# BetterBelle/eco-dqn

Measured on AMD Instinct MI355X. Metric: env-steps/sec (batched episodes) on ER-200 MaxCut, higher is better.
Workload: dtype f32-accurate MPNN on f16 MFMA (fp16x2: every operand a power-of-two-scaled pair of fp16 pieces, 22 significand bits, three products, f32 accumulate; aggregations and Linears alike; f32 MFMA on the CSR fallback) / f64+int (env)

## Files before the change

eco-dqn_amd/csrc/eco_train.hip:

```cpp
#include <cmath>

#include "eco_mpnn.h"
#include "eco_env_dev.h"

namespace eco {

struct WJob {
  const float* dY;
  const float* X1;
  const float* X2;
  int ld1, K1, ld2, K2;
  int R;
  int nO;
  int out_off;
  int out_ld;
  int out_col0;
};
constexpr int MAX_JOBS = 10;
#ifndef WGRAD_NT
#define WGRAD_NT 0
#endif
constexpr int WGRAD_WG_X = 3;
constexpr int WG_PER_JOB = 128;
constexpr int SLABS_PER_JOB = WG_PER_JOB;
constexpr int SLAB = 64 * 128;
constexpr int WROWS = 32;

struct WJobs {
  WJob j[MAX_JOBS];
  int n;
  int nwgj[MAX_JOBS];
  int first[MAX_JOBS + 1];
// ... 141 lines not shown
      if (rb + WROWS >= r1) break;
      store_tile(RB, rb + WROWS);
      __syncthreads();
      load_tile(RB, rb + 3 * WROWS);
      compute();
      __syncthreads();
    }
  }
  float* slab = slabs + ((size_t)jb * SLABS_PER_JOB + wg) * SLAB;
#pragma unroll
  for (int q = 0; q < 2; ++q) {
    const int t = w + 4 * q;
    if (t < ntile) {
      const int it = t >> 1;
#pragma unroll
      for (int k = 0; k < 16; ++k) {
        const int o = 32 * ot + (k & 3) + 8 * (k >> 2) + 4 * h;
        slab[o * 128 + 32 * it + jj] = acc[q][k];
      }
    }
  }
}

__global__ __launch_bounds__(256) void wgrad_bf3_kernel(WJobs jobs, float* slabs) {
  __shared__ __attribute__((aligned(16))) uint16_t sY[3 * 64 * WB_LD];
  __shared__ __attribute__((aligned(16))) uint16_t sX[3 * 128 * WB_LD];
  int jb = 0;
  while (jb + 1 < jobs.n && (int)blockIdx.x >= jobs.first[jb + 1]) ++jb;
  if (jobs.j[jb].K1 + jobs.j[jb].K2 > 64) wgrad_bf3_job<true>(jobs, slabs, jb, sY, sX);
  else wgrad_bf3_job<false>(jobs, slabs, jb, sY, sX);
}


__global__ void wgrad_reduce_kernel(WJobs jobs, const float* slabs, float* grad) {
  const WJob& J = jobs.j[blockIdx.y];
  const int K = J.K1 + J.K2;
  const int idx = blockIdx.x * blockDim.x + threadIdx.x;
  const int o = idx / 128, i = idx % 128;
  if (o >= J.nO || i >= K) return;
  const float* s = slabs + (size_t)blockIdx.y * SLABS_PER_JOB * SLAB + o * 128 + i;
  float acc = 0.f;
  const int nk = jobs.nwgj[blockIdx.y];
  int k = 0;
  for (; k + 8 <= nk; k += 8) {
    float v[8];
#pragma unroll
    for (int u = 0; u < 8; ++u) v[u] = s[(size_t)(k + u) * SLAB];
#pragma unroll
    for (int u = 0; u < 8; ++u) acc += v[u];
  }
  for (; k < nk; ++k) acc += s[(size_t)k * SLAB];
  grad[J.out_off + o * J.out_ld + J.out_col0 + i] = acc;
}

struct ColJob {
  const float* X;
  int R, ld, C;
  float* out;
  int out_stride;
};
struct ColJobs {
  ColJob j[4];
  int first[5];
};
__global__ void colsum_jobs_kernel(ColJobs jobs) {
  int jb = 0;
  while (jb < 3 && (int)blockIdx.x >= jobs.first[jb + 1]) ++jb;
  const ColJob& J = jobs.j[jb];
  __shared__ float red[256];
  const int c = (int)blockIdx.x - jobs.first[jb];
  float acc = 0.f;
  for (int r = threadIdx.x; r < J.R; r += 256) acc += J.X[(size_t)r * J.ld + c];
  red[threadIdx.x] = acc;
  __syncthreads();
  for (int s2 = 128; s2 > 0; s2 >>= 1) {
    if ((int)threadIdx.x < s2) red[threadIdx.x] += red[threadIdx.x + s2];
    __syncthreads();
  }
  if (threadIdx.x == 0) J.out[(size_t)c * J.out_stride] = red[0];
}

__global__ void td_kernel(const float* q_s, const float* q_tn, const int32_t* a_star, const int32_t* actions,
                          const float* rewards, const float* dones, int B, int N, float gamma, int clip,
                          float* dq, float* sqerr) {
  const size_t i = (size_t)blockIdx.x * blockDim.x + threadIdx.x;
  if (i >= (size_t)B * N) return;
  const int b = (int)(i / N), j = (int)(i - (size_t)b * N);
  int a = actions[b];
  if ((unsigned)a >= (unsigned)N) a = 0;
  if (j != a) {
    dq[i] = 0.f;
    return;
  }
  int as = a_star[b];
  if ((unsigned)as >= (unsigned)N) as = 0;
  float qt = q_tn[(size_t)b * N + as];
  if (clip && qt < 0.f) qt = 0.f;
  const float td = rewards[b] + (1.f - dones[b]) * gamma * qt;
  const float q = q_s[i];
  const float diff = q - td;
  dq[i] = 2.f * diff / (float)B;
  sqerr[b] = diff * diff;
}

__global__ void mean_kernel(const float* v, int n, float* out) {
  __shared__ float red[256];
  float acc = 0.f;
  for (int i = threadIdx.x; i < n; i += 256) acc += v[i];
  red[threadIdx.x] = acc;
  __syncthreads();
  for (int s = 128; s > 0; s >>= 1) {
    if ((int)threadIdx.x < s) red[threadIdx.x] += red[threadIdx.x + s];
    __syncthreads();
  }
  if (threadIdx.x == 0) *out = red[0] / (float)n;
}

__global__ void adam_kernel(float* p, const float* g, float* m, float* v, int n, float b1, float b2, float step_size,
                            float bc2_sqrt, float eps, float wd, float gscale) {
  const int i = blockIdx.x * blockDim.x + threadIdx.x;
  if (i >= n) return;
  float gi = gscale == 1.f ? g[i] : g[i] * gscale;
  if (wd != 0.f) gi = fmaf(wd, p[i], gi);
  const float mi = m[i] + (1.f - b1) * (gi - m[i]);
  const float vi = v[i] * b2 + (1.f - b2) * gi * gi;
  m[i] = mi;
  v[i] = vi;
  const float denom = sqrtf(vi) / bc2_sqrt + eps;
  p[i] = p[i] - step_size * (mi / denom);
}

__device__ __forceinline__ int xstride(const eco_replay& rb) { return rb.x_stride == 16 ? 16 : 8; }

__global__ void replay_push_kernel(eco_replay rb, int pos, int B, const float* xs, const float* xn,
                                   const int32_t* gids, const int32_t* actions, const double* rewards,
                                   const uint8_t* dones) {
  const int b = blockIdx.y;
  if (b >= B) return;
  const int slot = (int)(((long long)pos + b) % rb.capacity);
  const int per = rb.n_spins * xstride(rb) / 4;
  const float4* s4 = reinterpret_cast<const float4*>(xs + (size_t)b * rb.n_spins * xstride(rb));
  const float4* n4 = reinterpret_cast<const float4*>(xn + (size_t)b * rb.n_spins * xstride(rb));
  float4* ds = reinterpret_cast<float4*>(rb.xs + (size_t)slot * rb.n_spins * xstride(rb));
  float4* dn = reinterpret_cast<float4*>(rb.xn + (size_t)slot * rb.n_spins * xstride(rb));
  for (int i = blockIdx.x * blockDim.x + threadIdx.x; i < per; i += gridDim.x * blockDim.x) {
    ds[i] = s4[i];
    dn[i] = n4[i];
  }
  if (blockIdx.x == 0 && threadIdx.x == 0) {
    rb.gid[slot] = gids[b];
    rb.act[slot] = actions[b];
    rb.rew[slot] = (float)rewards[b];
    rb.done[slot] = dones[b] ? 1.f : 0.f;
  }
}

__device__ __forceinline__ uint32_t feistel(uint32_t x, int half, uint64_t key) {
  const uint32_t mask = (1u << half) - 1u;
  uint32_t L = x >> half, R = x & mask;
#pragma unroll
  for (int r = 0; r < 4; ++r) {
    const uint32_t F = (uint32_t)(rng3(key, (uint64_t)r, (uint64_t)R) & mask);
// ... 191 lines not shown
      const uint32_t tsfk = v == a ? 0u : (((w >> 16) & 0x7FFFu) + 1u) & 0x7FFFu;
      w = ((v == a ? ~w : w) & 0x80000000u) | (tsfk << 16) | (w & 0xFFFFu);
    }
    cr_lds[v] = w;
  }
  __syncthreads();
  if (flip) {
    const int32_t* rp = gs.row_ptr + (size_t)g * (N + 1);
    const uint32_t* ed = gs.edges + gs.edge_base[g];
    for (int q = rp[a] + threadIdx.x; q < rp[a + 1]; q += blockDim.x) {
      const uint32_t ex = ed[q];
      const int j = edge_col(ex);
      const uint32_t w = cr_lds[j];
      const int h = (int)(int16_t)(w & 0xFFFFu) - 2 * edge_w(ex) * sa_old;
      cr_lds[j] = (w & 0xFFFF0000u) | ((uint32_t)h & 0xFFFFu);
    }
    __syncthreads();
  }
  compact_expand(cfg, cr_lds, r.ctx_n + slot * 4, mlr, tab, N, xn + (size_t)m * N * W, red);
}

static size_t slab_bytes() { return (size_t)MAX_JOBS * SLABS_PER_JOB * SLAB * sizeof(float); }

}

using namespace eco;

extern "C" size_t eco_mpnn_backward_workspace_bytes(int32_t n_spins, int32_t batch) {
  const size_t g = mpnn_grad_ws_bytes(n_spins, batch);
  if (!g) return 0;
  return align_up(g, 256) + slab_bytes();
}

extern "C" int eco_mpnn_backward(const float* packed, int32_t n_obs_in, const eco_graph_set* gs,
                                 const int32_t* graph_ids, int32_t batch, const float* obs_x, const void* saved,
                                 const float* dq, float* grad, void* workspace, eco_stream_t stream) {
  if (!grad || !workspace) return fail(ECO_ERR_ARG, "null grad/workspace");
  hipStream_t st = (hipStream_t)stream;
  int rc = mpnn_backward_launch(packed, n_obs_in, gs, graph_ids, batch, obs_x, saved, dq, workspace, st);
  if (rc) return rc;
  const int N = gs->n_spins;
  const size_t RT = (size_t)batch * N;
  if (RT > (size_t)INT32_MAX / 64) return fail(ECO_ERR_ARG, "batch * n_spins too large");
  const float* sv = (const float*)saved;
  const float* gr = (const float*)workspace;
  auto SV = [&](int t) { return sv + (size_t)t * RT * 64; };
  auto GR = [&](int t) { return gr + (size_t)t * RT * 64; };
  const float* MEAN = sv + (size_t)SV_NODE_TENSORS * RT * 64;
  const float* DP = gr + (size_t)GR_NODE_TENSORS * RT * 64;
  const float* DWRA = DP + (size_t)batch * 64;
  const float* DWRB = DWRA + (size_t)batch * 64;
  const float* DBR = DWRB + (size_t)batch * 64;
  const float* DWA = DBR + (((size_t)batch + 63) & ~63ull);
  const int gpb = graphs_per_block(N, batch);
  const int nblk = (batch + gpb - 1) / gpb;
  float* slabs = (float*)((char*)workspace + align_up(mpnn_grad_ws_bytes(N, batch), 256));
  const FlatOffsets fo = flat_offsets(n_obs_in);
  WJobs J{};
  int n = 0;
  const int R = (int)RT;
  for (int l = 0; l < 3; ++l) {
    J.j[n++] = WJob{GR(GR_DUM0 + l), SV(SV_AGG0 + l), SV(SV_E), 64, 64, 64, 64, R, 64, fo.L + l * 16384, 128, 0};
    J.j[n++] = WJob{GR(GR_DUU0 + l), SV(SV_H0 + l), SV(SV_M0 + l), 64, 64, 64, 64, R, 64, fo.L + l * 16384 + 8192,
                    128, 0};
  }
  J.j[n++] = WJob{GR(GR_DUE), SV(SV_EAGG), nullptr, 64, 64, 0, 0, R, 64, fo.Wf, 64, 0};
  const int xw = ECO_OBS_X_STRIDE(n_obs_in);
  J.j[n++] = WJob{GR(GR_DU0), obs_x, nullptr, xw, n_obs_in, 0, 0, R, 64, fo.W0, n_obs_in, 0};
  J.j[n++] = WJob{GR(GR_DZ), obs_x, nullptr, xw, n_obs_in, 0, 0, R, 63, fo.We, 1 + n_obs_in, 1};
  J.j[n++] = WJob{DP, MEAN, nullptr, 64, 64, 0, 0, batch, 64, fo.Wp, 64, 0};
  J.n = n;
  {
    const int total = WGRAD_WG_X * 256;
    double rows = 0.0;
    for (int j = 0; j < n; ++j) rows += J.j[j].R;
    J.first[0] = 0;
    for (int j = 0; j < n; ++j) {
      const int g = (int)(total * (double)J.j[j].R / rows);
      J.nwgj[j] = std::max(1, std::min(WG_PER_JOB, g));
      J.first[j + 1] = J.first[j] + J.nwgj[j];
    }
    wgrad_bf3_kernel<<<J.first[n], 256, 0, st>>>(J, slabs);
  }
  wgrad_reduce_kernel<<<dim3(64 * 128 / 256, n), 256, 0, st>>>(J, slabs, grad);
  ColJobs CJ{};
  CJ.j[0] = ColJob{DWRA, batch, 64, 64, grad + fo.Wr, 1};
  CJ.j[1] = ColJob{DWRB, batch, 64, 64, grad + fo.Wr + 64, 1};
  CJ.j[2] = ColJob{DBR, batch, 1, 1, grad + fo.Br, 1};
  CJ.j[3] = ColJob{DWA, nblk, 64, 63, grad + fo.We, 1 + n_obs_in};
  CJ.first[0] = 0;
  for (int k = 0; k < 4; ++k) CJ.first[k + 1] = CJ.first[k] + CJ.j[k].C;
  colsum_jobs_kernel<<<CJ.first[4], 256, 0, st>>>(CJ);
  return check_launch("mpnn_backward_wgrad");
}

extern "C" int eco_dqn_td(const float* q_s, const float* q_target_next, const int32_t* a_star,
                          const int32_t* actions, const float* rewards, const float* dones, int32_t batch,
                          int32_t n_spins, float gamma, int32_t clip_q_targets, float* dq, float* sqerr,
                          float* loss, eco_stream_t stream) {
  if (!q_s || !q_target_next || !a_star || !actions || !rewards || !dones || !dq || !sqerr || !loss)
    return fail(ECO_ERR_ARG, "null argument");
  if (batch < 1 || n_spins < 1) return fail(ECO_ERR_ARG, "bad batch/n_spins");
  hipStream_t st = (hipStream_t)stream;
  const size_t n = (size_t)batch * n_spins;
  td_kernel<<<(unsigned)((n + 255) / 256), 256, 0, st>>>(q_s, q_target_next, a_star, actions, rewards, dones, batch,
                                                         n_spins, gamma, clip_q_targets, dq, sqerr);
  mean_kernel<<<1, 256, 0, st>>>(sqerr, batch, loss);
  return check_launch("dqn_td");
}

extern "C" int eco_adam(float* params, const float* grad, float* exp_avg, float* exp_avg_sq, int32_t n, double lr,
                        double beta1, double beta2, double eps, double weight_decay, double grad_scale, int64_t step,
                        eco_stream_t stream) {
  if (!params || !grad || !exp_avg || !exp_avg_sq || n < 1 || step < 1) return fail(ECO_ERR_ARG, "bad adam args");
  const double bc1 = 1.0 - std::pow(beta1, (double)step);
  const double bc2 = 1.0 - std::pow(beta2, (double)step);
  adam_kernel<<<(n + 255) / 256, 256, 0, (hipStream_t)stream>>>(params, grad, exp_avg, exp_avg_sq, n, (float)beta1,
                                                               (float)beta2, (float)(lr / bc1),
                                                               (float)std::sqrt(bc2), (float)eps,
                                                               (float)weight_decay, (float)grad_scale);
  return check_launch("adam");
}

extern "C" int eco_replay_push(const eco_replay* rb, int32_t pos, int32_t batch, const float* xs, const float* xn,
                               const int32_t* graph_ids, const int32_t* actions, const double* rewards,
                               const uint8_t* dones, eco_stream_t stream) {
  if (!rb || !xs || !xn || !graph_ids || !actions || !rewards || !dones) return fail(ECO_ERR_ARG, "null argument");
  if (rb->x_stride != 0 && rb->x_stride != 8 && rb->x_stride != 16) return fail(ECO_ERR_ARG, "x_stride must be 8 or 16");
  if (batch < 1 || rb->capacity < 1 || pos < 0) return fail(ECO_ERR_ARG, "bad batch/capacity/pos");
  if (batch > rb->capacity) return fail(ECO_ERR_ARG, "replay push: batch larger than the ring (slots would collide)");
  replay_push_kernel<<<dim3(1, batch), 256, 0, (hipStream_t)stream>>>(*rb, pos, batch, xs, xn, graph_ids, actions,
                                                                      rewards, dones);
  return check_launch("replay_push");
}

extern "C" int eco_replay_sample(const eco_replay* rb, int32_t size, int32_t m, uint64_t seed, uint64_t counter,
                                 float* xs, float* xn, int32_t* graph_ids, int32_t* actions, float* rewards,
                                 float* dones, eco_stream_t stream) {
  if (!rb || !xs || !xn || !graph_ids || !actions || !rewards || !dones) return fail(ECO_ERR_ARG, "null argument");
  if (rb->x_stride != 0 && rb->x_stride != 8 && rb->x_stride != 16) return fail(ECO_ERR_ARG, "x_stride must be 8 or 16");
  if (size < m || m < 1 || size > rb->capacity)
    return fail(ECO_ERR_ARG, "replay sample: need m <= size <= capacity (random.sample without replacement)");
  replay_sample_kernel<<<dim3(1, m), 256, 0, (hipStream_t)stream>>>(*rb, size, m, rng3(seed, counter, 0x5A5A),
                                                                    xs, xn, graph_ids, actions, rewards, dones);
  return check_launch("replay_sample");
}

static int compact_check(const eco_env_config* cfg, int32_t batch, int32_t capacity) {
  if (!cfg) return fail(ECO_ERR_ARG, "null config");
  if (cfg->optimisation_target != ECO_TARGET_CUT) return fail(ECO_ERR_TARGET, "compact replay: OptimisationTarget.CUT only");
  if (cfg->float_weights)
    return fail(ECO_ERR_ARG, "compact replay: integer weights only (its local field is an int16); a float-weighted "
                             "env uses the feature ring (eco_replay_push / eco_replay_sample)");
// ... 61 lines not shown
```

eco-dqn_amd/eco_hip/_lib.py:

```python
import ctypes
import os

_HERE = os.path.dirname(os.path.abspath(__file__))
LIB_PATH = os.environ.get("ECO_HIP_LIB", os.path.join(_HERE, "libecohip.so"))

if not os.path.exists(LIB_PATH):
    raise ImportError(f"libecohip.so not found at {LIB_PATH}: build it with `make -C eco-dqn_amd` "
                      "(hipcc --offload-arch=gfx950); eco_hip has no fallback path")
lib = ctypes.CDLL(LIB_PATH)

ECO_OK, ECO_ERR_ARG, ECO_ERR_HIP, ECO_ERR_PAST_END, ECO_ERR_BASIS, ECO_ERR_TARGET, ECO_ERR_OBSERVABLE, \
    ECO_ERR_GRAPH, ECO_ERR_KEY, ECO_ERR_INDEX = range(10)
ECO_MAX_OBS = 16
ECO_MPNN_MAX_OBS = 16
ECO_ENV_SCALARS = 16
ECO_TARGET_CUT, ECO_TARGET_ENERGY, ECO_TARGET_MIN_COVER, ECO_TARGET_MIN_CUT, ECO_TARGET_MAX_IND_SET, \
    ECO_TARGET_MAX_CLIQUE, ECO_TARGET_MIN_DOM_SET = range(1, 8)


def obs_x_stride(n_obs):
    return 8 if n_obs <= 8 else 16
ECO_MAX_SPINS = 2048
ECO_COMPACT_MAX_SPINS = 8192
ECO_NORM_PER_GRAPH, ECO_NORM_PER_CALL, ECO_NORM_PER_CALL_REUSE = 0, 1, 2
ECO_GRAPH_ER, ECO_GRAPH_BA = 1, 2
ECO_WEIGHTS_UNIFORM, ECO_WEIGHTS_DISCRETE, ECO_WEIGHTS_RANDOM = 0, 1, 2
ECO_PATH_NO_DENSE, ECO_PATH_NO_DL, ECO_PATH_NO_SHARED, ECO_PATH_NO_PAIR, ECO_PATH_DENSE2_FWD = 1, 2, 4, 8, 16


class EnvConfig(ctypes.Structure):
    _fields_ = [("n_spins", ctypes.c_int32), ("max_steps", ctypes.c_int32), ("n_obs", ctypes.c_int32),
                ("obs_ids", ctypes.c_int32 * ECO_MAX_OBS), ("reward_signal", ctypes.c_int32),
                ("norm_rewards", ctypes.c_int32), ("reversible_spins", ctypes.c_int32),
                ("spin_basis", ctypes.c_int32), ("stopping", ctypes.c_int32),
                ("has_basin_reward", ctypes.c_int32), ("has_stag_punishment", ctypes.c_int32),
                ("horizon_length", ctypes.c_int32), ("optimisation_target", ctypes.c_int32),
                ("basin_reward", ctypes.c_double),
                ("stag_punishment", ctypes.c_double), ("float_weights", ctypes.c_int32)]


class GraphSet(ctypes.Structure):
    _fields_ = [("n_graphs", ctypes.c_int32), ("n_spins", ctypes.c_int32), ("row_ptr", ctypes.c_void_p),
                ("edge_base", ctypes.c_void_p), ("edges", ctypes.c_void_p), ("deg", ctypes.c_void_p),
                ("max_deg", ctypes.c_void_p), ("meta", ctypes.c_void_p), ("valid", ctypes.c_void_p),
                ("unit_weights", ctypes.c_int32), ("adjbits", ctypes.c_void_p),
                ("edge_weights", ctypes.c_void_p)]


class Replay(ctypes.Structure):
    _fields_ = [("capacity", ctypes.c_int32), ("n_spins", ctypes.c_int32), ("x_stride", ctypes.c_int32),
                ("xs", ctypes.c_void_p),
                ("xn", ctypes.c_void_p), ("gid", ctypes.c_void_p), ("act", ctypes.c_void_p),
                ("rew", ctypes.c_void_p), ("done", ctypes.c_void_p)]


class ActConfig(ctypes.Structure):
    _fields_ = [("epsilon", ctypes.c_float), ("reversible", ctypes.c_int32), ("allowed_value", ctypes.c_float),
                ("seed", ctypes.c_uint64), ("counter", ctypes.c_uint64)]


_P = ctypes.c_void_p
_I = ctypes.c_int32
_SIG = {
    "eco_graphs_prepare": (ctypes.c_int, [ctypes.POINTER(GraphSet), _P]),
    "eco_graphs_adjbits_bytes": (ctypes.c_size_t, [_I, _I]),
    "eco_graphs_generate_workspace_bytes": (ctypes.c_size_t, [_I, _I]),
    "eco_graphs_generate": (ctypes.c_int, [ctypes.POINTER(GraphSet), _I, _I, _I, ctypes.c_double, _I,
                                           ctypes.c_uint64, ctypes.c_int64, _P, _P]),
    "eco_env_state_bytes": (ctypes.c_size_t, [ctypes.POINTER(EnvConfig), _I]),
    "eco_env_reset": (ctypes.c_int, [ctypes.POINTER(EnvConfig), ctypes.POINTER(GraphSet), _P, _I, _P, _P, _P,
                                     ctypes.c_uint64, _P, _P, _P]),
    "eco_env_step": (ctypes.c_int, [ctypes.POINTER(EnvConfig), ctypes.POINTER(GraphSet), _P, _I, _P, _P, _P, _P,
                                    _P, _P]),
    "eco_env_read": (ctypes.c_int, [ctypes.POINTER(EnvConfig), _P, _I, _P, _P, _P, _P]),
    "eco_check_errors": (ctypes.c_int, [_P]),
    "eco_error_word_copy": (ctypes.c_int, [_P, _P]),
    "eco_set_kernel_paths": (_I, [_I]),
    "eco_probe_split2_mfma": (ctypes.c_int, [_P, _P, _P, _I, _I, _P, _P]),
    "eco_env_greedy_actions": (ctypes.c_int, [ctypes.POINTER(EnvConfig), ctypes.POINTER(GraphSet), _P, _I, _P,
                                              _P]),
    "eco_mpnn_param_count": (ctypes.c_size_t, [_I]),
    "eco_mpnn_packed_count": (ctypes.c_size_t, []),
    "eco_mpnn_pack": (ctypes.c_int, [_P, _I, _P, _P]),
    "eco_mpnn_workspace_bytes": (ctypes.c_size_t, [_I, _I]),
    "eco_mpnn_forward": (ctypes.c_int, [_P, _I, ctypes.POINTER(GraphSet), _P, _I, _P, _I, _P,
                                        ctypes.POINTER(ActConfig), _P, _P, _P, _P]),
    "eco_mpnn_forward_pair": (ctypes.c_int, [_P, _P, _I, ctypes.POINTER(GraphSet), _P, _I, _P, _I, _P,
                                             ctypes.POINTER(ActConfig), _P, _P, ctypes.POINTER(ActConfig), _P, _P,
                                             _P]),
    "eco_mpnn_saved_bytes": (ctypes.c_size_t, [_I, _I]),
    "eco_mpnn_backward_workspace_bytes": (ctypes.c_size_t, [_I, _I]),
    "eco_mpnn_backward": (ctypes.c_int, [_P, _I, ctypes.POINTER(GraphSet), _P, _I, _P, _P, _P, _P, _P, _P]),
    "eco_dqn_td": (ctypes.c_int, [_P, _P, _P, _P, _P, _P, _I, _I, ctypes.c_float, _I, _P, _P, _P, _P]),
    "eco_adam": (ctypes.c_int, [_P, _P, _P, _P, _I, ctypes.c_double, ctypes.c_double, ctypes.c_double,
                                ctypes.c_double, ctypes.c_double, ctypes.c_double, ctypes.c_int64, _P]),
    "eco_replay_push": (ctypes.c_int, [ctypes.POINTER(Replay), _I, _I, _P, _P, _P, _P, _P, _P, _P]),
    "eco_replay_sample": (ctypes.c_int, [ctypes.POINTER(Replay), _I, _I, ctypes.c_uint64, ctypes.c_uint64, _P, _P,
                                         _P, _P, _P, _P, _P]),
    "eco_replay_compact_bytes": (ctypes.c_size_t, [_I, _I, _I]),
    "eco_replay_compact_snapshot": (ctypes.c_int, [ctypes.POINTER(EnvConfig), _P, _I, _P, _I, ctypes.c_int64, _P,
                                                   _P]),
    "eco_replay_compact_push": (ctypes.c_int, [ctypes.POINTER(EnvConfig), _P, _I, _P, _I, ctypes.c_int64, _P, _P, _P,
                                               _P]),
    "eco_replay_compact_sample": (ctypes.c_int, [ctypes.POINTER(EnvConfig), _P, ctypes.POINTER(GraphSet), _I, _P, _I,
                                                 _I, ctypes.c_int64, _I, ctypes.c_uint64, ctypes.c_uint64, _P, _P, _P, _P, _P, _P,
                                                 _P]),
    "eco_per_create": (_P, [_I, ctypes.c_double, ctypes.c_double]),
    "eco_per_destroy": (None, [_P]),
    "eco_per_len": (_I, [_P]),
    "eco_per_beta": (ctypes.c_double, [_P]),
    "eco_per_full": (ctypes.c_int, [_P]),
    "eco_per_configure_beta_anneal_time": (ctypes.c_int, [_P, ctypes.c_double]),
    "eco_per_add": (ctypes.c_int, [_P, _I, _P]),
    "eco_per_update_priorities": (ctypes.c_int, [_P, _I, _P, _P]),
    "eco_per_rebalance": (ctypes.c_int, [_P]),
    "eco_per_sample": (ctypes.c_int, [_P, _I, _P, ctypes.c_uint64, _P, _P, _P]),
    "eco_per_sample_begin": (ctypes.c_int, [_P, _I, _P]),
    "eco_per_sample_finish": (ctypes.c_int, [_P, _I, _P, ctypes.c_uint64, _P, _P, _P]),
    "eco_per_heap": (ctypes.c_int, [_P, _P, _P]),
    "eco_per_partitions": (_I, [_P, _P, _P]),
    "eco_replay_gather": (ctypes.c_int, [ctypes.POINTER(Replay), _I, _P, _P, _P, _P, _P, _P, _P, _P]),
    "eco_last_error": (ctypes.c_char_p, []),
}
for _name, (_res, _args) in _SIG.items():
    _f = getattr(lib, _name)
# ... 18 lines not shown
    if rc == ECO_ERR_BASIS:
        raise Exception(msg)
    if rc == ECO_ERR_HIP:
        raise RuntimeError(msg)
    if rc == ECO_ERR_KEY:
        raise KeyError(msg)
    if rc == ECO_ERR_INDEX:
        raise IndexError(msg)
    raise ValueError(msg)


def ptr(t):
    return None if t is None else ctypes.c_void_p(t.data_ptr())


def stream_ptr(stream=None):
    import torch
    s = stream if stream is not None else torch.cuda.current_stream()
    return ctypes.c_void_p(s.cuda_stream)


class kernel_paths:

    def __init__(self, mask):
        self.mask = int(mask)

    def __enter__(self):
        self.prev = lib.eco_set_kernel_paths(self.mask)
        return self

    def __exit__(self, *exc):
        lib.eco_set_kernel_paths(self.prev)
        return False
```

eco-dqn_amd/eco_hip/agents/dqn/dqn.py:

```python
import ctypes
import math
import os
import random

import numpy as np
import torch

from ... import _lib
from ...parallel import allreduce_gradients_async, broadcast_parameters
from .utils import CompactReplayBuffer, ReplayBuffer, TestMetric, set_global_seed


def graph_slots_needed(n_envs, max_steps, replay_buffer_size):
    per_batch = n_envs * max_steps
    return n_envs * (-(-int(replay_buffer_size) // per_batch) + 1)


class DQN:
    def __init__(self, envs, network, init_network_params=None, init_weight_std=None, double_dqn=True,
                 update_target_frequency=10000, gamma=0.99, clip_Q_targets=False, replay_start_size=50000,
                 replay_buffer_size=1000000, minibatch_size=32, update_frequency=1, update_learning_rate=True,
                 initial_learning_rate=0, peak_learning_rate=1e-3, peak_learning_rate_step=10000,
                 final_learning_rate=5e-5, final_learning_rate_step=200000, max_grad_norm=None, weight_decay=0,
                 update_exploration=True, initial_exploration_rate=1, final_exploration_rate=0.1,
# ... 170 lines not shown
                                                                       device=self.device)
        self.network.forward_graphs(obs_x, self.graphs, graph_ids, norm_scope=_lib.ECO_NORM_PER_GRAPH,
                                    act=self._act_config(eps), actions_out=out)
        return out

    @torch.no_grad()
    def predict(self, obs_x, graph_ids, graphs=None, norm_scope=_lib.ECO_NORM_PER_CALL):
        out = torch.empty(obs_x.shape[0], dtype=torch.int32, device=self.device)
        self.network.forward_graphs(obs_x, graphs or self.graphs, graph_ids, norm_scope=norm_scope,
                                    act=self._act_config(0.0), actions_out=out)
        return out

    def train_step(self, transitions, sync_loss=True, loss_out=None, overlap=None):
        xs, act, rew, xn, done, gid = transitions
        loss_dev = self.loss_dev if loss_out is None else loss_out
        m = xs.shape[0]
        if m != self._train_m:
            self._alloc_train_buffers(m)
        net, tgt = self.network, self.target_network
        greedy = _lib.ActConfig(0.0, int(self.acting_in_reversible_spin_env), float(self.allowed_value), 0, 0)
        if self.double_dqn:
            net.forward_pair_graphs(tgt, xn, self.graphs, gid, norm_scope=_lib.ECO_NORM_PER_CALL, act=greedy,
                                    actions_out=self.a_star, q_out_other=self.q_tn)
            scope_s = _lib.ECO_NORM_PER_CALL_REUSE
        else:
            tgt.forward_graphs(xn, self.graphs, gid, norm_scope=_lib.ECO_NORM_PER_CALL, q_out=self.q_tn,
                               act=greedy, actions_out=self.a_star)
            scope_s = _lib.ECO_NORM_PER_CALL
        net.forward_graphs(xs, self.graphs, gid, norm_scope=scope_s, q_out=self.q_s, saved=self.saved)
        _lib.check(_lib.lib.eco_dqn_td(_lib.ptr(self.q_s), _lib.ptr(self.q_tn), _lib.ptr(self.a_star),
                                       _lib.ptr(act), _lib.ptr(rew), _lib.ptr(done), m, self.N,
                                       ctypes.c_float(self.gamma), int(bool(self.clip_Q_targets)), _lib.ptr(self.dq),
                                       _lib.ptr(self.sqerr), _lib.ptr(loss_dev), _lib.stream_ptr()))
        net.backward_graphs(xs, self.graphs, gid, self.saved, self.dq, self.grad, workspace=self.bw_ws)
        work, scale = allreduce_gradients_async(self.grad)
        if overlap is not None:
            overlap()
        if work is not None:
            work.wait()
        self.adam_step += 1
        _lib.check(_lib.lib.eco_adam(_lib.ptr(net.flat), _lib.ptr(self.grad), _lib.ptr(self.exp_avg),
                                     _lib.ptr(self.exp_avg_sq), net.flat.numel(), self.lr, 0.9, 0.999,
                                     self.adam_epsilon, float(self.weight_decay), scale, self.adam_step,
                                     _lib.stream_ptr()))
        net.repack()
        self.grad_steps += 1
        self._samples_since_sync += m * self.world
        if sync_loss:
            return loss_dev.item()
        return loss_dev if loss_out is not None else loss_dev.clone()

    def sync_target(self):
        self.target_network.flat.copy_(self.network.flat)

    def _take_graph_slots(self, episodes):
        k = self.B if episodes is None else int(episodes.sum())
        if self.regenerate_graphs is None:
            ids = self.graph_pool_ids[self._rng.integers(0, len(self.graph_pool_ids), k)]
            if episodes is None:
                return ids
            out = np.zeros(self.B, np.int64)
            out[episodes] = ids
            return out
        kind, param = self.regenerate_graphs[:2]
        weights = (self.regenerate_graphs[2] if len(self.regenerate_graphs) > 2
                   else "random" if self.graphs.float_weights else "discrete")
        n_slots = len(self._slot_users)
        if self._started:
            old = self._host_graph_ids
            old = old if episodes is None else old[episodes]
            np.subtract.at(self._slot_users, old, 1)
            self._slot_free_at[old[self._slot_users[old] == 0]] = self._pushed
        ids = (self._slot_cursor + np.arange(k)) % n_slots
        self._slot_cursor = int((self._slot_cursor + k) % n_slots)
        safe = (self._slot_users[ids] == 0) & (self._pushed - self._slot_free_at[ids] >= self.replay_buffer_size)
        fresh = ids[safe]
        for run in np.split(fresh, np.nonzero(np.diff(fresh) != 1)[0] + 1) if len(fresh) else []:
# ... 525 lines not shown
```

eco-dqn_amd/eco_hip/networks/mpnn.py:

```python
import ctypes

import numpy as np
import torch

from .. import _lib
from ..graphs import GraphStore, dense_to_csr

N_FEATURES = 64


def param_layout(n_obs_in=7):
    lay = [("node_init_embedding_layer.0.weight", (64, n_obs_in)),
           ("edge_embedding_layer.edge_embedding_NN.weight", (63, n_obs_in + 1)),
           ("edge_embedding_layer.edge_feature_NN.weight", (64, 64))]
    for i in range(3):
        lay.append((f"update_node_embedding_layer.{i}.message_layer.weight", (64, 128)))
        lay.append((f"update_node_embedding_layer.{i}.update_layer.weight", (64, 128)))
    lay += [("readout_layer.layer_pooled.weight", (64, 64)),
            ("readout_layer.layers_readout.0.weight", (1, 128)),
            ("readout_layer.layers_readout.0.bias", (1,))]
    return lay


class MPNN(torch.nn.Module):
# ... 97 lines not shown

    def forward_pair_graphs(self, other, obs_x, graphs, graph_ids, norm_scope=_lib.ECO_NORM_PER_GRAPH, q_out=None,
                            act=None, actions_out=None, q_out_other=None, act_other=None, actions_out_other=None,
                            stream=None):
        B, N = obs_x.shape[0], obs_x.shape[1]
        self._check_x(obs_x)
        if other.n_obs_in != self.n_obs_in:
            raise ValueError("paired networks must take the same observables")
        self._ensure_packed(stream)
        other._ensure_packed(stream)
        if q_out is None and act is None:
            q_out = torch.empty(B, N, dtype=torch.float32, device=obs_x.device)
        if q_out_other is None and act_other is None:
            q_out_other = torch.empty(B, N, dtype=torch.float32, device=obs_x.device)
        gids = graph_ids if graph_ids.dtype == torch.int32 else graph_ids.to(torch.int32)
        if self.timer is not None:
            ev = (torch.cuda.Event(enable_timing=True), torch.cuda.Event(enable_timing=True))
            ev[0].record()
        _lib.check(_lib.lib.eco_mpnn_forward_pair(
            _lib.ptr(self.packed), _lib.ptr(other.packed), self.n_obs_in, ctypes.byref(graphs.gs),
            _lib.ptr(gids.contiguous()), B, _lib.ptr(obs_x), norm_scope, _lib.ptr(q_out),
            ctypes.byref(act) if act is not None else None, _lib.ptr(actions_out), _lib.ptr(q_out_other),
            ctypes.byref(act_other) if act_other is not None else None, _lib.ptr(actions_out_other),
            _lib.ptr(self._workspace(N, B)), _lib.stream_ptr(stream)))
        if self.timer is not None:
            ev[1].record()
            self.timer.append((ev[0], ev[1], 2 * B, graph_ids))
        return q_out, q_out_other

    @staticmethod
    def saved_bytes(n_spins, batch):
        return _lib.lib.eco_mpnn_saved_bytes(n_spins, batch)

    def backward_graphs(self, obs_x, graphs, graph_ids, saved, dq, grad_out, workspace=None, stream=None):
        B, N = obs_x.shape[0], obs_x.shape[1]
        self._check_x(obs_x)
        need = _lib.lib.eco_mpnn_backward_workspace_bytes(N, B)
        if workspace is None or workspace.numel() < need:
            workspace = torch.empty(need, dtype=torch.uint8, device=obs_x.device)
        gids = graph_ids if graph_ids.dtype == torch.int32 else graph_ids.to(torch.int32)
        if self.timer is not None:
            ev = (torch.cuda.Event(enable_timing=True), torch.cuda.Event(enable_timing=True))
            ev[0].record()
        _lib.check(_lib.lib.eco_mpnn_backward(
            _lib.ptr(self.packed), self.n_obs_in, ctypes.byref(graphs.gs), _lib.ptr(gids.contiguous()), B,
            _lib.ptr(obs_x), _lib.ptr(saved), _lib.ptr(dq), _lib.ptr(grad_out), _lib.ptr(workspace),
            _lib.stream_ptr(stream)))
        if self.timer is not None:
            ev[1].record()
            self.timer.append((ev[0], ev[1], -B, graph_ids))
        return grad_out

    def forward(self, obs):
        if obs.dim() == 2:
            view = obs.unsqueeze(0)
        else:
            view = obs
        B, R, N = view.shape
        k = self.n_obs_in
        x = torch.zeros(B, N, _lib.obs_x_stride(k), dtype=torch.float32, device=self.flat.device)
        x[:, :, :k] = view[:, :k, :].transpose(1, 2).to(x.device, torch.float32)
        adj = view[:, k:, :].detach().cpu().numpy()
        store = GraphStore.from_csr(dense_to_csr([a.T for a in adj]), device=self.flat.device)
        gids = torch.arange(B, dtype=torch.int32, device=self.flat.device)
        q = self.forward_graphs(x, store, gids, norm_scope=_lib.ECO_NORM_PER_CALL)
        if obs.dim() == 3:
            obs.transpose_(-1, -2)
        return q.squeeze()
```

include/eco_hip.h:

```cpp
#ifndef ECO_HIP_H
#define ECO_HIP_H

#include <stddef.h>
#include <stdint.h>

#ifdef __cplusplus
extern "C" {
#endif

typedef void *eco_stream_t;

enum {
  ECO_OK = 0,
  ECO_ERR_ARG = 1,
  ECO_ERR_HIP = 2,
  ECO_ERR_PAST_END = 3,
  ECO_ERR_BASIS = 4,
  ECO_ERR_TARGET = 5,
  ECO_ERR_OBSERVABLE = 6,
  ECO_ERR_GRAPH = 7,
  ECO_ERR_KEY = 8,
  ECO_ERR_INDEX = 9
};

// ... 86 lines not shown
       ECO_NORM_PER_CALL_REUSE = 2  };

typedef struct {
  float epsilon;
  int32_t reversible;
  float allowed_value;
  uint64_t seed;
  uint64_t counter;
} eco_act_config;

size_t eco_mpnn_workspace_bytes(int32_t n_spins, int32_t batch);
size_t eco_mpnn_saved_bytes(int32_t n_spins, int32_t batch);

int eco_mpnn_forward(const float *packed, int32_t n_obs_in, const eco_graph_set *gs, const int32_t *graph_ids,
                     int32_t batch, const float *obs_x, int32_t norm_scope, float *q, const eco_act_config *act,
                     int32_t *actions, void *saved, void *workspace, eco_stream_t stream);

int eco_mpnn_forward_pair(const float *packed_a, const float *packed_b, int32_t n_obs_in, const eco_graph_set *gs,
                          const int32_t *graph_ids, int32_t batch, const float *obs_x, int32_t norm_scope,
                          float *q_a, const eco_act_config *act_a, int32_t *actions_a, float *q_b,
                          const eco_act_config *act_b, int32_t *actions_b, void *workspace, eco_stream_t stream);

enum { ECO_PATH_NO_DENSE = 1, ECO_PATH_NO_DL = 2, ECO_PATH_NO_SHARED = 4, ECO_PATH_NO_PAIR = 8, ECO_PATH_DENSE2_FWD = 16 };
int32_t eco_set_kernel_paths(int32_t mask);

int eco_probe_split2_mfma(const float *x, const float *sf, const uint16_t *w_frags, int32_t n_blocks, int32_t order,
                          float *out, eco_stream_t stream);


size_t eco_mpnn_backward_workspace_bytes(int32_t n_spins, int32_t batch);
int eco_mpnn_backward(const float *packed, int32_t n_obs_in, const eco_graph_set *gs, const int32_t *graph_ids,
                      int32_t batch, const float *obs_x, const void *saved, const float *dq, float *grad,
                      void *workspace, eco_stream_t stream);

int eco_dqn_td(const float *q_s, const float *q_target_next, const int32_t *a_star, const int32_t *actions,
               const float *rewards, const float *dones, int32_t batch, int32_t n_spins, float gamma,
               int32_t clip_q_targets, float *dq, float *sqerr, float *loss, eco_stream_t stream);

int eco_adam(float *params, const float *grad, float *exp_avg, float *exp_avg_sq, int32_t n, double lr,
             double beta1, double beta2, double eps, double weight_decay, double grad_scale, int64_t step,
             eco_stream_t stream);

typedef struct {
  int32_t capacity;
  int32_t n_spins;
  int32_t x_stride;
  float *xs;
  float *xn;
  int32_t *gid;
  int32_t *act;
  float *rew;
  float *done;
} eco_replay;

int eco_replay_push(const eco_replay *rb, int32_t pos, int32_t batch, const float *xs, const float *xn,
                    const int32_t *graph_ids, const int32_t *actions, const double *rewards, const uint8_t *dones,
                    eco_stream_t stream);
int eco_replay_sample(const eco_replay *rb, int32_t size, int32_t m, uint64_t seed, uint64_t counter, float *xs,
                      float *xn, int32_t *graph_ids, int32_t *actions, float *rewards, float *dones,
                      eco_stream_t stream);

#define ECO_COMPACT_MAX_SPINS 8192
size_t eco_replay_compact_bytes(int32_t n_spins, int32_t capacity, int32_t batch);
int eco_replay_compact_snapshot(const eco_env_config *cfg, const void *env_state, int32_t batch, void *ring,
                                int32_t capacity, int64_t pushed, const uint8_t *mask, eco_stream_t stream);
int eco_replay_compact_push(const eco_env_config *cfg, const void *env_state, int32_t batch, void *ring,
// ... 37 lines not shown
```

Baseline: 437,400.

## Fuse weight-gradient reduce, column sums and Adam update into one tail kernel

Merges the slab reduction, column-sum and Adam optimizer kernels at the end of the backward pass into a single launch. Each gradient element gets its Adam update right after it is reduced, which removes two kernel launches and a re-read of the gradient buffer. The fused path is used only when no distributed process group is initialized; the multi-device path keeps the separate allreduce and Adam. This assumes every parameter is covered by exactly one reduce or colsum output, since any parameter not written there would never receive its Adam update.

```diff
diff --git a/eco-dqn_amd/csrc/eco_train.hip b/eco-dqn_amd/csrc/eco_train.hip
--- a/eco-dqn_amd/csrc/eco_train.hip
+++ b/eco-dqn_amd/csrc/eco_train.hip
@@ -1,3 +1,4 @@
+#include <atomic>
 #include <cmath>
 
 #include "eco_mpnn.h"
@@ -205,15 +206,33 @@
 }
 
 
-__global__ void wgrad_reduce_kernel(WJobs jobs, const float* slabs, float* grad) {
-  const WJob& J = jobs.j[blockIdx.y];
+struct AdamArgs {
+  float *p, *m, *v;
+  float b1, b2, step_size, bc2_sqrt, eps, wd, gscale;
+};
+__device__ __forceinline__ void adam_elem(const AdamArgs& A, int i, float g) {
+  asm volatile("" : "+v"(g));
+  float gi = A.gscale == 1.f ? g : g * A.gscale;
+  if (A.wd != 0.f) gi = fmaf(A.wd, A.p[i], gi);
+  const float mi = A.m[i] + (1.f - A.b1) * (gi - A.m[i]);
+  const float vi = A.v[i] * A.b2 + (1.f - A.b2) * gi * gi;
+  A.m[i] = mi;
+  A.v[i] = vi;
+  const float denom = sqrtf(vi) / A.bc2_sqrt + A.eps;
+  A.p[i] = A.p[i] - A.step_size * (mi / denom);
+}
+
+__device__ __forceinline__ void wgrad_reduce_block(const WJobs& jobs, const float* slabs, float* grad, int jb, int bx,
+                                                   const AdamArgs& A) {
+  const WJob& J = jobs.j[jb];
   const int K = J.K1 + J.K2;
-  const int idx = blockIdx.x * blockDim.x + threadIdx.x;
+  const int idx = bx * 256 + threadIdx.x;
   const int o = idx / 128, i = idx % 128;
   if (o >= J.nO || i >= K) return;
-  const float* s = slabs + (size_t)blockIdx.y * SLABS_PER_JOB * SLAB + o * 128 + i;
+  const int dst = J.out_off + o * J.out_ld + J.out_col0 + i;
+  const float* s = slabs + (size_t)jb * SLABS_PER_JOB * SLAB + o * 128 + i;
   float acc = 0.f;
-  const int nk = jobs.nwgj[blockIdx.y];
+  const int nk = jobs.nwgj[jb];
   int k = 0;
   for (; k + 8 <= nk; k += 8) {
     float v[8];
@@ -223,7 +242,12 @@
     for (int u = 0; u < 8; ++u) acc += v[u];
   }
   for (; k < nk; ++k) acc += s[(size_t)k * SLAB];
-  grad[J.out_off + o * J.out_ld + J.out_col0 + i] = acc;
+  grad[dst] = acc;
+  if (A.p) adam_elem(A, dst, acc);
+}
+
+__global__ void wgrad_reduce_kernel(WJobs jobs, const float* slabs, float* grad) {
+  wgrad_reduce_block(jobs, slabs, grad, blockIdx.y, blockIdx.x, AdamArgs{});
 }
 
 struct ColJob {
@@ -236,12 +260,12 @@
   ColJob j[4];
   int first[5];
 };
-__global__ void colsum_jobs_kernel(ColJobs jobs) {
+__device__ __forceinline__ void colsum_block(const ColJobs& jobs, int bx, float* grad, const AdamArgs& A) {
   int jb = 0;
-  while (jb < 3 && (int)blockIdx.x >= jobs.first[jb + 1]) ++jb;
+  while (jb < 3 && bx >= jobs.first[jb + 1]) ++jb;
   const ColJob& J = jobs.j[jb];
   __shared__ float red[256];
-  const int c = (int)blockIdx.x - jobs.first[jb];
+  const int c = bx - jobs.first[jb];
   float acc = 0.f;
   for (int r = threadIdx.x; r < J.R; r += 256) acc += J.X[(size_t)r * J.ld + c];
   red[threadIdx.x] = acc;
@@ -250,7 +274,21 @@
     if ((int)threadIdx.x < s2) red[threadIdx.x] += red[threadIdx.x + s2];
     __syncthreads();
   }
-  if (threadIdx.x == 0) J.out[(size_t)c * J.out_stride] = red[0];
+  if (threadIdx.x == 0) {
+    float* dst = J.out + (size_t)c * J.out_stride;
+    const float g = red[0];
+    *dst = g;
+    if (A.p) adam_elem(A, (int)(dst - grad), g);
+  }
+}
+__global__ void colsum_jobs_kernel(ColJobs jobs) { colsum_block(jobs, (int)blockIdx.x, nullptr, AdamArgs{}); }
+
+constexpr int REDUCE_BLOCKS = 64 * 128 / 256;
+__global__ __launch_bounds__(256) void wgrad_tail_kernel(WJobs jobs, const float* slabs, float* grad, ColJobs cj,
+                                                         AdamArgs A) {
+  const int b = (int)blockIdx.x, nred = REDUCE_BLOCKS * jobs.n;
+  if (b < nred) wgrad_reduce_block(jobs, slabs, grad, b / REDUCE_BLOCKS, b % REDUCE_BLOCKS, A);
+  else colsum_block(cj, b - nred, grad, A);
 }
 
 __global__ void td_kernel(const float* q_s, const float* q_tn, const int32_t* a_star, const int32_t* actions,
@@ -289,18 +327,10 @@
   if (threadIdx.x == 0) *out = red[0] / (float)n;
 }
 
-__global__ void adam_kernel(float* p, const float* g, float* m, float* v, int n, float b1, float b2, float step_size,
-                            float bc2_sqrt, float eps, float wd, float gscale) {
+__global__ void adam_kernel(AdamArgs A, const float* g, int n) {
   const int i = blockIdx.x * blockDim.x + threadIdx.x;
   if (i >= n) return;
-  float gi = gscale == 1.f ? g[i] : g[i] * gscale;
-  if (wd != 0.f) gi = fmaf(wd, p[i], gi);
-  const float mi = m[i] + (1.f - b1) * (gi - m[i]);
-  const float vi = v[i] * b2 + (1.f - b2) * gi * gi;
-  m[i] = mi;
-  v[i] = vi;
-  const float denom = sqrtf(vi) / bc2_sqrt + eps;
-  p[i] = p[i] - step_size * (mi / denom);
+  adam_elem(A, i, g[i]);
 }
 
 __device__ __forceinline__ int xstride(const eco_replay& rb) { return rb.x_stride == 16 ? 16 : 8; }
@@ -558,10 +588,25 @@
   return align_up(g, 256) + slab_bytes();
 }
 
-extern "C" int eco_mpnn_backward(const float* packed, int32_t n_obs_in, const eco_graph_set* gs,
-                                 const int32_t* graph_ids, int32_t batch, const float* obs_x, const void* saved,
-                                 const float* dq, float* grad, void* workspace, eco_stream_t stream) {
+static std::atomic<int> g_train_tail{0};
+
+extern "C" int32_t eco_set_train_tail(int32_t mask) {
+  return g_train_tail.exchange(mask & ECO_TAIL_SPLIT_LAUNCHES);
+}
+
+static AdamArgs adam_args(float* params, float* exp_avg, float* exp_avg_sq, double lr, double beta1, double beta2,
+                          double eps, double weight_decay, double grad_scale, int64_t step) {
+  const double bc1 = 1.0 - std::pow(beta1, (double)step);
+  const double bc2 = 1.0 - std::pow(beta2, (double)step);
+  return AdamArgs{params, exp_avg, exp_avg_sq, (float)beta1, (float)beta2, (float)(lr / bc1), (float)std::sqrt(bc2),
+                  (float)eps, (float)weight_decay, (float)grad_scale};
+}
+
+static int backward_impl(const float* packed, int32_t n_obs_in, const eco_graph_set* gs, const int32_t* graph_ids,
+                         int32_t batch, const float* obs_x, const void* saved, const float* dq, float* grad,
+                         void* workspace, const AdamArgs& A, eco_stream_t stream) {
   if (!grad || !workspace) return fail(ECO_ERR_ARG, "null grad/workspace");
+  const int tail = g_train_tail.load(std::memory_order_relaxed);
   hipStream_t st = (hipStream_t)stream;
   int rc = mpnn_backward_launch(packed, n_obs_in, gs, graph_ids, batch, obs_x, saved, dq, workspace, st);
   if (rc) return rc;
@@ -608,7 +653,6 @@
     }
     wgrad_bf3_kernel<<<J.first[n], 256, 0, st>>>(J, slabs);
   }
-  wgrad_reduce_kernel<<<dim3(64 * 128 / 256, n), 256, 0, st>>>(J, slabs, grad);
   ColJobs CJ{};
   CJ.j[0] = ColJob{DWRA, batch, 64, 64, grad + fo.Wr, 1};
   CJ.j[1] = ColJob{DWRB, batch, 64, 64, grad + fo.Wr + 64, 1};
@@ -616,8 +660,30 @@
   CJ.j[3] = ColJob{DWA, nblk, 64, 63, grad + fo.We, 1 + n_obs_in};
   CJ.first[0] = 0;
   for (int k = 0; k < 4; ++k) CJ.first[k + 1] = CJ.first[k] + CJ.j[k].C;
-  colsum_jobs_kernel<<<CJ.first[4], 256, 0, st>>>(CJ);
+  if (tail & ECO_TAIL_SPLIT_LAUNCHES) {
+    wgrad_reduce_kernel<<<dim3(REDUCE_BLOCKS, n), 256, 0, st>>>(J, slabs, grad);
+    colsum_jobs_kernel<<<CJ.first[4], 256, 0, st>>>(CJ);
+    if (A.p) adam_kernel<<<(fo.total + 255) / 256, 256, 0, st>>>(A, grad, fo.total);
+  } else {
+    wgrad_tail_kernel<<<REDUCE_BLOCKS * n + CJ.first[4], 256, 0, st>>>(J, slabs, grad, CJ, A);
+  }
   return check_launch("mpnn_backward_wgrad");
+}
+
+extern "C" int eco_mpnn_backward(const float* packed, int32_t n_obs_in, const eco_graph_set* gs,
+                                 const int32_t* graph_ids, int32_t batch, const float* obs_x, const void* saved,
+                                 const float* dq, float* grad, void* workspace, eco_stream_t stream) {
+  return backward_impl(packed, n_obs_in, gs, graph_ids, batch, obs_x, saved, dq, grad, workspace, AdamArgs{}, stream);
+}
+
+extern "C" int eco_mpnn_backward_adam(const float* packed, int32_t n_obs_in, const eco_graph_set* gs,
+                                      const int32_t* graph_ids, int32_t batch, const float* obs_x, const void* saved,
+                                      const float* dq, float* grad, void* workspace, float* params, float* exp_avg,
+                                      float* exp_avg_sq, double lr, double beta1, double beta2, double eps,
+                                      double weight_decay, int64_t step, eco_stream_t stream) {
+  if (!params || !exp_avg || !exp_avg_sq || step < 1) return fail(ECO_ERR_ARG, "bad adam args");
+  return backward_impl(packed, n_obs_in, gs, graph_ids, batch, obs_x, saved, dq, grad, workspace,
+                       adam_args(params, exp_avg, exp_avg_sq, lr, beta1, beta2, eps, weight_decay, 1.0, step), stream);
 }
 
 extern "C" int eco_dqn_td(const float* q_s, const float* q_target_next, const int32_t* a_star,
@@ -639,12 +705,8 @@
                         double beta1, double beta2, double eps, double weight_decay, double grad_scale, int64_t step,
                         eco_stream_t stream) {
   if (!params || !grad || !exp_avg || !exp_avg_sq || n < 1 || step < 1) return fail(ECO_ERR_ARG, "bad adam args");
-  const double bc1 = 1.0 - std::pow(beta1, (double)step);
-  const double bc2 = 1.0 - std::pow(beta2, (double)step);
-  adam_kernel<<<(n + 255) / 256, 256, 0, (hipStream_t)stream>>>(params, grad, exp_avg, exp_avg_sq, n, (float)beta1,
-                                                               (float)beta2, (float)(lr / bc1),
-                                                               (float)std::sqrt(bc2), (float)eps,
-                                                               (float)weight_decay, (float)grad_scale);
+  adam_kernel<<<(n + 255) / 256, 256, 0, (hipStream_t)stream>>>(
+      adam_args(params, exp_avg, exp_avg_sq, lr, beta1, beta2, eps, weight_decay, grad_scale, step), grad, n);
   return check_launch("adam");
 }
 
diff --git a/eco-dqn_amd/eco_hip/_lib.py b/eco-dqn_amd/eco_hip/_lib.py
--- a/eco-dqn_amd/eco_hip/_lib.py
+++ b/eco-dqn_amd/eco_hip/_lib.py
@@ -26,6 +26,7 @@
 ECO_GRAPH_ER, ECO_GRAPH_BA = 1, 2
 ECO_WEIGHTS_UNIFORM, ECO_WEIGHTS_DISCRETE, ECO_WEIGHTS_RANDOM = 0, 1, 2
 ECO_PATH_NO_DENSE, ECO_PATH_NO_DL, ECO_PATH_NO_SHARED, ECO_PATH_NO_PAIR, ECO_PATH_DENSE2_FWD = 1, 2, 4, 8, 16
+ECO_TAIL_SPLIT_LAUNCHES = 1
 
 
 class EnvConfig(ctypes.Structure):
@@ -91,6 +92,10 @@
     "eco_mpnn_saved_bytes": (ctypes.c_size_t, [_I, _I]),
     "eco_mpnn_backward_workspace_bytes": (ctypes.c_size_t, [_I, _I]),
     "eco_mpnn_backward": (ctypes.c_int, [_P, _I, ctypes.POINTER(GraphSet), _P, _I, _P, _P, _P, _P, _P, _P]),
+    "eco_mpnn_backward_adam": (ctypes.c_int, [_P, _I, ctypes.POINTER(GraphSet), _P, _I, _P, _P, _P, _P, _P, _P, _P, _P,
+                                              ctypes.c_double, ctypes.c_double, ctypes.c_double, ctypes.c_double,
+                                              ctypes.c_double, ctypes.c_int64, _P]),
+    "eco_set_train_tail": (_I, [_I]),
     "eco_dqn_td": (ctypes.c_int, [_P, _P, _P, _P, _P, _P, _I, _I, ctypes.c_float, _I, _P, _P, _P, _P]),
     "eco_adam": (ctypes.c_int, [_P, _P, _P, _P, _I, ctypes.c_double, ctypes.c_double, ctypes.c_double,
                                 ctypes.c_double, ctypes.c_double, ctypes.c_double, ctypes.c_int64, _P]),
@@ -175,3 +180,17 @@
     def __exit__(self, *exc):
         lib.eco_set_kernel_paths(self.prev)
         return False
+
+
+class train_tail:
+
+    def __init__(self, mask):
+        self.mask = int(mask)
+
+    def __enter__(self):
+        self.prev = lib.eco_set_train_tail(self.mask)
+        return self
+
+    def __exit__(self, *exc):
+        lib.eco_set_train_tail(self.prev)
+        return False
diff --git a/eco-dqn_amd/eco_hip/agents/dqn/dqn.py b/eco-dqn_amd/eco_hip/agents/dqn/dqn.py
--- a/eco-dqn_amd/eco_hip/agents/dqn/dqn.py
+++ b/eco-dqn_amd/eco_hip/agents/dqn/dqn.py
@@ -226,17 +226,24 @@
                                        _lib.ptr(act), _lib.ptr(rew), _lib.ptr(done), m, self.N,
                                        ctypes.c_float(self.gamma), int(bool(self.clip_Q_targets)), _lib.ptr(self.dq),
                                        _lib.ptr(self.sqerr), _lib.ptr(loss_dev), _lib.stream_ptr()))
-        net.backward_graphs(xs, self.graphs, gid, self.saved, self.dq, self.grad, workspace=self.bw_ws)
-        work, scale = allreduce_gradients_async(self.grad)
-        if overlap is not None:
-            overlap()
-        if work is not None:
-            work.wait()
         self.adam_step += 1
-        _lib.check(_lib.lib.eco_adam(_lib.ptr(net.flat), _lib.ptr(self.grad), _lib.ptr(self.exp_avg),
-                                     _lib.ptr(self.exp_avg_sq), net.flat.numel(), self.lr, 0.9, 0.999,
-                                     self.adam_epsilon, float(self.weight_decay), scale, self.adam_step,
-                                     _lib.stream_ptr()))
+        if not (torch.distributed.is_available() and torch.distributed.is_initialized()):
+            net.backward_graphs(xs, self.graphs, gid, self.saved, self.dq, self.grad, workspace=self.bw_ws,
+                                adam=(self.exp_avg, self.exp_avg_sq, self.lr, 0.9, 0.999, self.adam_epsilon,
+                                      float(self.weight_decay), self.adam_step))
+            if overlap is not None:
+                overlap()
+        else:
+            net.backward_graphs(xs, self.graphs, gid, self.saved, self.dq, self.grad, workspace=self.bw_ws)
+            work, scale = allreduce_gradients_async(self.grad)
+            if overlap is not None:
+                overlap()
+            if work is not None:
+                work.wait()
+            _lib.check(_lib.lib.eco_adam(_lib.ptr(net.flat), _lib.ptr(self.grad), _lib.ptr(self.exp_avg),
+                                         _lib.ptr(self.exp_avg_sq), net.flat.numel(), self.lr, 0.9, 0.999,
+                                         self.adam_epsilon, float(self.weight_decay), scale, self.adam_step,
+                                         _lib.stream_ptr()))
         net.repack()
         self.grad_steps += 1
         self._samples_since_sync += m * self.world
diff --git a/eco-dqn_amd/eco_hip/networks/mpnn.py b/eco-dqn_amd/eco_hip/networks/mpnn.py
--- a/eco-dqn_amd/eco_hip/networks/mpnn.py
+++ b/eco-dqn_amd/eco_hip/networks/mpnn.py
@@ -153,7 +153,8 @@
     def saved_bytes(n_spins, batch):
         return _lib.lib.eco_mpnn_saved_bytes(n_spins, batch)
 
-    def backward_graphs(self, obs_x, graphs, graph_ids, saved, dq, grad_out, workspace=None, stream=None):
+    def backward_graphs(self, obs_x, graphs, graph_ids, saved, dq, grad_out, workspace=None, stream=None,
+                        adam=None):
         B, N = obs_x.shape[0], obs_x.shape[1]
         self._check_x(obs_x)
         need = _lib.lib.eco_mpnn_backward_workspace_bytes(N, B)
@@ -163,10 +164,18 @@
         if self.timer is not None:
             ev = (torch.cuda.Event(enable_timing=True), torch.cuda.Event(enable_timing=True))
             ev[0].record()
-        _lib.check(_lib.lib.eco_mpnn_backward(
-            _lib.ptr(self.packed), self.n_obs_in, ctypes.byref(graphs.gs), _lib.ptr(gids.contiguous()), B,
-            _lib.ptr(obs_x), _lib.ptr(saved), _lib.ptr(dq), _lib.ptr(grad_out), _lib.ptr(workspace),
-            _lib.stream_ptr(stream)))
+        if adam is None:
+            _lib.check(_lib.lib.eco_mpnn_backward(
+                _lib.ptr(self.packed), self.n_obs_in, ctypes.byref(graphs.gs), _lib.ptr(gids.contiguous()), B,
+                _lib.ptr(obs_x), _lib.ptr(saved), _lib.ptr(dq), _lib.ptr(grad_out), _lib.ptr(workspace),
+                _lib.stream_ptr(stream)))
+        else:
+            exp_avg, exp_avg_sq, lr, beta1, beta2, eps, weight_decay, step = adam
+            _lib.check(_lib.lib.eco_mpnn_backward_adam(
+                _lib.ptr(self.packed), self.n_obs_in, ctypes.byref(graphs.gs), _lib.ptr(gids.contiguous()), B,
+                _lib.ptr(obs_x), _lib.ptr(saved), _lib.ptr(dq), _lib.ptr(grad_out), _lib.ptr(workspace),
+                _lib.ptr(self.flat), _lib.ptr(exp_avg), _lib.ptr(exp_avg_sq), lr, beta1, beta2, eps, weight_decay,
+                step, _lib.stream_ptr(stream)))
         if self.timer is not None:
             ev[1].record()
             self.timer.append((ev[0], ev[1], -B, graph_ids))
diff --git a/include/eco_hip.h b/include/eco_hip.h
--- a/include/eco_hip.h
+++ b/include/eco_hip.h
@@ -142,6 +142,14 @@
 int eco_mpnn_backward(const float *packed, int32_t n_obs_in, const eco_graph_set *gs, const int32_t *graph_ids,
                       int32_t batch, const float *obs_x, const void *saved, const float *dq, float *grad,
                       void *workspace, eco_stream_t stream);
+
+int eco_mpnn_backward_adam(const float *packed, int32_t n_obs_in, const eco_graph_set *gs, const int32_t *graph_ids,
+                           int32_t batch, const float *obs_x, const void *saved, const float *dq, float *grad,
+                           void *workspace, float *params, float *exp_avg, float *exp_avg_sq, double lr, double beta1,
+                           double beta2, double eps, double weight_decay, int64_t step, eco_stream_t stream);
+
+enum { ECO_TAIL_SPLIT_LAUNCHES = 1 };
+int32_t eco_set_train_tail(int32_t mask);
 
 int eco_dqn_td(const float *q_s, const float *q_target_next, const int32_t *a_star, const int32_t *actions,
                const float *rewards, const float *dones, int32_t batch, int32_t n_spins, float gamma,
```

Result: no change. 439,200, median of 6 (+0.4%).
